# zubair-irshad/NeRF-MAE

Measured on AMD Instinct MI355X. Metric: voxel-grids/sec (fwd+bwd+optimizer) swin_s 160^3 bf16, higher is better.
Workload: dtype bf16; 1 GPU; swin_s MAE pretraining step, global batch 8 = 8 grid(s)/GPU of 4x160^3 RGB-sigma, mask_ratio 0.75, stochastic depth 0.1, AdamW+clip, DP=1 (BASELINE configs[2], the headline, read literally); global_batch=8, grids_per_gpu=8, resolution=160, parallelism=dp1, launch=hipgraph

## Files before the change

include/nerfmae_hip.h:

```cpp
#ifndef NERFMAE_HIP_H
#define NERFMAE_HIP_H
#include <stdint.h>
#ifdef __cplusplus
extern "C" {
#endif
#define NMH_API __attribute__((visibility("default")))

NMH_API int nmh_version(void);
NMH_API const char* nmh_error_string(int code);

NMH_API int nmh_gemm_nt(int dt, const void* A, int64_t lda, const void* W, int64_t ldw, int M, int N, int K, void* C, int64_t ldc, const float* bias, int act, void* C2, const void* resid, const float* rowscale, int rows_per_scale, int accumulate, void* stream);
NMH_API int nmh_gemm_nt_window_scatter(int dt, const void* A, int64_t lda, const void* W, int64_t ldw, int M, int N, int K, void* out, const void* resid, const float* bias, const float* rowscale, int tokens_per_sample, const int* wm, void* stream);
NMH_API int nmh_gemm_tn(int dt, const void* A, int64_t lda, const void* B, int64_t ldb, float* dW, int64_t M, int N, int K, const float* rowscale, int rows_per_scale, int omode, int64_t ldo, int p0, int p1, float* dbias, float* ws, int64_t ws_floats, void* stream);
typedef struct nmh_tn_problem { const void* A; int64_t lda; const void* B; int64_t ldb; float* dW; int64_t ldo; float* dbias; const float* rowscale; int64_t M; int N; int K; int rows_per_sample;
  int64_t stride_k; int up_k; int up_v; int bias_atomic; int n_inner; int64_t stride_n2; } nmh_tn_problem;
NMH_API int nmh_gemm_tn_grouped(int dt, const nmh_tn_problem* probs, int nprob, float* ws, int64_t ws_floats, void* stream);
NMH_API int nmh_gemm_tn_grouped_fg(int dt, const nmh_tn_problem* probs, int nprob, float* ws, int64_t ws_floats, void* stream);
NMH_API int nmh_conv3d_k3(int dt, const void* X, const void* Wp, void* Y, int B, int D, int H, int W, int Cin, int Cout, int accumulate, float* ws, int64_t ws_floats, void* stream);
NMH_API int nmh_conv3d_k3_bias(int dt, const void* X, const void* Wp, const float* bias, void* Y, int B, int D, int H, int W, int Cin, int Cout, void* stream);
NMH_API int nmh_nearest_upsample_add(int dt, const void* coarse, void* fine, int B, int Dc, int Hc, int Wc, int Df, int Hf, int Wf, int C, void* stream);
NMH_API int nmh_nearest_upsample_add_bwd(int dt, const void* dfine, void* dcoarse, int B, int Dc, int Hc, int Wc, int Df, int Hf, int Wf, int C, void* stream);
NMH_API int nmh_copy_cols(int dt, const void* src, int64_t lds, void* dst, int64_t ldd, int64_t M, int C, void* stream);
NMH_API int nmh_ndhwc_to_ncdhw(int dt, const void* src, float* dst, int B, int64_t V, int C, void* stream);
NMH_API int nmh_ncdhw_to_ndhwc(int dt, const float* src, void* dst, int B, int64_t V, int C, void* stream);
NMH_API int nmh_conv3d_k3_c48(const void* X, const void* Wk, void* Y, int B, int D, int H, int W, int accumulate, double* stats_acc, void* stream);
NMH_API int nmh_conv3d_k3_c48_bwd_reduce(const void* dY, const void* Wkd, void* dX, int B, int D, int H, int W, const void* Y1, const float* stats1, float slope, double* sums, void* stream);
NMH_API int nmh_conv3d_k3_c48mb(const void* X, const void* Wk, void* Y, int B, int D, int H, int W, int Cin, int Cout, int accumulate, void* stream);
NMH_API int nmh_conv3d_k3_c64(const void* X, const void* Wk, void* Y, int B, int D, int H, int W, int Cin, int Cout, int accumulate, double* stats_acc, const float* bias, void* stream);
NMH_API int64_t nmh_conv3d_k3_c64_pack_numel(int Cin, int Cout);
NMH_API int nmh_conv3d_k3_c64_wgrad(const void* dY, const void* X, float* dW, float* ws, int B, int D, int H, int W, int Cin, int Cout, void* stream);
NMH_API int64_t nmh_conv3d_k3_c64_wgrad_ws_floats(void);
NMH_API int nmh_instnorm_finalize(const double* acc, float* stats, int B, int64_t V, int C, float eps, void* stream);
NMH_API int nmh_conv3d_k3_c48_wgrad(const void* dY, const void* X, float* dW, float* ws, int B, int D, int H, int W, void* stream);
NMH_API int nmh_conv3d_k3_wgrad_halo(const void* dY, const void* X, float* dW, float* ws, int B, int D, int H, int W, int Cin, int Cout, void* stream);
NMH_API int64_t nmh_conv3d_k3_c48_wgrad_ws_floats(void);
NMH_API int nmh_conv3d_k3_wgrad(int dt, const void* dY, const void* X, float* dW, int B, int D, int H, int W, int Cin, int Cout, void* stream);

NMH_API int nmh_layernorm_fwd(int dt, int src_mode, const void* x, void* out, const float* gamma, const float* beta, float eps, float* mean, float* rstd, int64_t rows, int C, const int* wm, const float* pos, const unsigned char* mask, const float* mask_token, int64_t tokens_per_sample, void* stream);
NMH_API int nmh_layernorm_bwd(int dt, int src_mode, const void* dy, const void* x, const float* gamma, const float* mean, const float* rstd, const void* dres, void* dx, float* dgamma, float* dbeta, int64_t rows, int C, const int* wm, const unsigned char* mask, float* dmask_token, int64_t tokens_per_sample, void* dyw, const float* dyw_scale, void* stream);
typedef struct nmh_ln_reduce_item { const float* partials; float* dgamma; float* dbeta; int64_t partial_rows; int C; int reserved; } nmh_ln_reduce_item;
NMH_API int64_t nmh_layernorm_bwd_partial_rows(int64_t rows, int C);
NMH_API int nmh_layernorm_bwd_deferred(int dt, int src_mode, const void* dy, const void* x, const float* gamma, const float* mean, const float* rstd, const void* dres, void* dx, float* partials, int64_t rows, int C, const int* wm, void* dyw, const float* dyw_scale, int64_t tokens_per_sample, void* stream);
NMH_API int nmh_layernorm_param_grad_reduce(const nmh_ln_reduce_item* items, int n, void* stream);
NMH_API int64_t nmh_cconv_pack_numel(void);
NMH_API int64_t nmh_cconv_pack_ws_floats(void);
NMH_API int nmh_cconv_pack(const float* Wt, const float* W1, const float* bt, void* Wcp, float* delta, float* ws, void* stream);
NMH_API int nmh_cconv_fwd(const void* x, const void* Wcp, const float* delta, void* y1, int B, int v, double* stats_acc, void* stream);
NMH_API int nmh_cconv_pack_centered(const float* Wt, const float* W1, const float* bt, void* Wcp, float* delta, float* ws, float* mean_table, void* stream);
NMH_API int nmh_cconv_output_mean(const void* x, const float* mean_table, const float* delta, double* class_sums, float* mean, int B, int v, void* stream);
NMH_API int nmh_conv48_pack_scaled(const float* W, const float* stats, void* Wk_per_sample, int B, void* stream);
// ... 165 lines not shown
```

nerf-mae_amd/csrc/capi.hip:

```cpp
#include "../../include/nerfmae_hip.h"
#include "kernels.hpp"
#include <cstdio>

static inline WinMap to_wm(const int* w) {
  WinMap m{};
  if (w) { m.B = w[0]; m.H = w[1]; m.W = w[2]; m.D = w[3]; m.PH = w[4]; m.PW = w[5]; m.PD = w[6]; m.s0 = w[7]; m.s1 = w[8]; m.s2 = w[9]; }
  return m;
}
#define ST ((hipStream_t)stream)
#define NMH_DT_BF16_C 1
#define REQ(...) do { const void* req_[] = {__VA_ARGS__}; for (const void* q_ : req_) if (!q_) return -4; } while (0)
#define CLR() (void)hipGetLastError()

extern "C" {
int nmh_version(void) { return 100; }
const char* nmh_error_string(int code) {
  if (code == 0) return "ok";
  if (code == -1) return "nmh: unsupported operation";
  if (code == -2) return "nmh: shape constraint violated (channel counts must be multiples of 8; head_dim must be 32)";
  if (code == -3) return "nmh: row too wide for the layernorm kernels";
  if (code < 0) return "nmh: invalid argument";
  return hipGetErrorString((hipError_t)code);
}
int nmh_gemm_nt(int dt, const void* A, int64_t lda, const void* W, int64_t ldw, int M, int N, int K, void* C, int64_t ldc, const float* bias, int act, void* C2,
// ... 6 lines not shown
}
int nmh_gemm_nt_window_scatter(int dt, const void* A, int64_t lda, const void* W, int64_t ldw, int M, int N, int K, void* out, const void* resid, const float* bias,
                               const float* rowscale, int tokens_per_sample, const int* wm, void* stream) {
  CLR();
  REQ(A, W, out, resid, wm);
  if (M <= 0) return 0;
  EpiParams ep{out, N, bias, 0, nullptr, resid, rowscale, tokens_per_sample > 0 ? tokens_per_sample : 1, 0};
  ep.win_on = 1; ep.wm = to_wm(wm);
  return k_gemm_nt(dt, A, lda, W, ldw, M, N, K, ep, ST);
}
int nmh_gemm_tn(int dt, const void* A, int64_t lda, const void* B, int64_t ldb, float* dW, int64_t M, int N, int K, const float* rowscale, int rows_per_scale,
                int omode, int64_t ldo, int p0, int p1, float* dbias, float* ws, int64_t ws_floats, void* stream) {
  CLR();
  REQ(A, B, dW);
  if (M <= 0) return 0;
  TnGeom gm{};
  gm.omode = omode; gm.ldo = ldo; gm.dbias = dbias; gm.ws = ws; gm.ws_floats = ws ? (long)ws_floats : 0;
  if (omode == 2) { gm.Cin = p0; gm.V = (unsigned)p1; gm.dC = make_fdiv(p0); }
  return k_gemm_tn(dt, A, lda, B, ldb, dW, M, N, K, rowscale, rows_per_scale > 0 ? rows_per_scale : 1, gm, ST);
}
int nmh_gemm_tn_grouped(int dt, const nmh_tn_problem* probs, int nprob, float* ws, int64_t ws_floats, void* stream) {
  CLR();
  if (nprob <= 0) return 0;
  if (dt != NMH_DT_BF16_C || probs == nullptr) return -4;
  static_assert(sizeof(nmh_tn_problem) == sizeof(TnProblemHost), "descriptor layouts must agree");
  return k_gemm_tn_grouped(reinterpret_cast<const TnProblemHost*>(probs), nprob, ws, ws ? (long)ws_floats : 0, ST);
}
int nmh_gemm_tn_grouped_fg(int dt, const nmh_tn_problem* probs, int nprob, float* ws, int64_t ws_floats, void* stream) {
  CLR();
  if (nprob <= 0) return 0;
  if (dt != NMH_DT_BF16_C || probs == nullptr) return -4;
  return k_gemm_tn_grouped(reinterpret_cast<const TnProblemHost*>(probs), nprob, ws, ws ? (long)ws_floats : 0, ST, true);
}
int nmh_upconv_fwd(int dt, const void* x, const void* Wt, const float* bias, void* cat, int64_t ldc, int B, int v, int k, int Cin, int Cout, void* stream) {
  CLR();
  REQ(x, Wt, cat);
  return k_upconv_fwd(dt, x, Wt, bias, cat, (long)ldc, B, v, k, Cin, Cout, ST);
}
int nmh_upconv_dgrad(int dt, const void* dcat, int64_t ldc, const void* Wd, void* dx, int B, int v, int k, int Cin, int Cout, void* stream) {
  CLR();
  REQ(dcat, Wd, dx);
  return k_upconv_dgrad(dt, dcat, (long)ldc, Wd, dx, B, v, k, Cin, Cout, ST);
}
int nmh_upconv_wgrad(int dt, const void* dcat, int64_t ldc, const void* x, float* dW, float* dbias, int B, int v, int k, int Cin, int Cout, void* stream) {
  CLR();
  REQ(dcat, x, dW);
  return k_upconv_wgrad(dt, dcat, (long)ldc, x, dW, dbias, B, v, k, Cin, Cout, ST);
}
int nmh_conv3d_k3(int dt, const void* X, const void* Wp, void* Y, int B, int D, int H, int W, int Cin, int Cout, int accumulate, float* ws, int64_t ws_floats, void* stream) {
  CLR();
  REQ(X, Wp, Y);
  EpiParams ep{Y, Cout, nullptr, 0, nullptr, nullptr, nullptr, 1, accumulate};
  return k_conv3_nt(dt, X, Wp, B, D, H, W, Cin, Cout, ep, ST, ws, ws ? (long)ws_floats : 0);
}
int nmh_conv3d_k3_bias(int dt, const void* X, const void* Wp, const float* bias, void* Y, int B, int D, int H, int W, int Cin, int Cout, void* stream) {
  CLR();
  REQ(X, Wp, bias, Y);
  EpiParams ep{Y, Cout, bias, 0, nullptr, nullptr, nullptr, 1, 0};
  return k_conv3_nt(dt, X, Wp, B, D, H, W, Cin, Cout, ep, ST);
}
int nmh_conv3d_k3_c64(const void* X, const void* Wk, void* Y, int B, int D, int H, int W, int Cin, int Cout, int accumulate, double* stats_acc, const float* bias, void* stream) {
  CLR();
  if (!X || !Wk || !Y) return -4;
  return k_conv64(X, Wk, Y, B, D, H, W, Cin, Cout, accumulate, stats_acc, bias, ST);
}
int nmh_conv3d_k3_c64_wgrad(const void* dY, const void* X, float* dW, float* ws, int B, int D, int H, int W, int Cin, int Cout, void* stream) {
  CLR();
// ... 946 lines not shown
```

nerf-mae_amd/csrc/kernels.hpp:

```cpp
#pragma once
#include <hip/hip_runtime.h>

struct FDiv { unsigned M; int sh; unsigned d; };
FDiv make_fdiv(unsigned d);

struct WinMap { int B, H, W, D, PH, PW, PD, s0, s1, s2; };

struct EpiParams {
  void* C; long ldc;
  const float* bias;
  int act; void* C2;
  const void* resid;
  const float* rowscale; int rows_per_scale;
  int accumulate;
  int up_k, up_v, up_cout;
  FDiv up_dv, up_dk, up_dc;
  int win_on; WinMap wm;
  int ksplit; int nbatch; float* kpart;
};

struct TnGeom {
  int omode;
  long ldo;
  int Cin, D, H, W; unsigned V;
// ... 30 lines not shown
  const int x = (int)(tu - q * (unsigned)w.D);
  unsigned q2 = q / (unsigned)w.W;
  const int y = (int)(q - q2 * (unsigned)w.W);
  const unsigned b = q2 / (unsigned)w.H;
  const int z = (int)(q2 - b * (unsigned)w.H);
  int pz = z - w.s0, py = y - w.s1, px = x - w.s2;
  if (pz < 0) pz += w.PH;
  if (py < 0) py += w.PW;
  if (px < 0) px += w.PD;
  const unsigned win = ((b * ((unsigned)w.PH >> 2) + ((unsigned)pz >> 2)) * ((unsigned)w.PW >> 2) + ((unsigned)py >> 2)) * ((unsigned)w.PD >> 2) + ((unsigned)px >> 2);
  return (long)win * 64 + ((pz & 3) << 4) + ((py & 3) << 2) + (px & 3);
}

#endif
int k_gemm_nt(int dt, const void* A, long lda, const void* Bw, long ldb, int M, int N, int K, const EpiParams& ep, hipStream_t st);
int k_upconv_fwd(int dt, const void* x, const void* Wt, const float* bias, void* cat, long ldc, int B, int v, int k, int Cin, int Cout, hipStream_t st);
int k_upconv_dgrad(int dt, const void* dcat, long ldc, const void* Wd, void* dx, int B, int v, int k, int Cin, int Cout, hipStream_t st);
int k_upconv_wgrad(int dt, const void* dcat, long ldc, const void* x, float* dW, float* dbias, int B, int v, int k, int Cin, int Cout, hipStream_t st);
int k_conv3_nt(int dt, const void* X, const void* Wp, int B, int D, int H, int W, int Cin, int Cout, const EpiParams& ep, hipStream_t st, float* ws = nullptr, long ws_floats = 0);
int k_gemm_tn(int dt, const void* A, long lda, const void* Bm, long ldb, float* Out, long M, int N, int K, const float* rowscale, int rows_per_scale, const TnGeom& gm, hipStream_t st);
struct TnProblemHost {
  const void* A; long lda;
  const void* B; long ldb;
  float* dW; long ldo;
  float* dbias;
  const float* rowscale;
  long M; int N, K; int rows_per_sample;
  long stride_k;
  int up_k, up_v;
  int bias_atomic;
  int n_inner; long stride_n2;
};
int k_gemm_tn_grouped(const TnProblemHost* probs, int nprob, float* ws, long ws_floats, hipStream_t st, bool foreground = false);
int k_conv48(const void* X, const void* Wk, void* Y, int B, int D, int H, int W, int accumulate, double* stats_acc, hipStream_t st,
             const void* Y1 = nullptr, const float* stats1 = nullptr, float slope = 0.f, long wk_sample_stride = 0, int centered = 0);
int k_conv48_pack_scaled(const float* W, const float* stats, void* out, int B, hipStream_t st);
int k_conv48_mb(const void* X, const void* Wk, void* Y, int B, int D, int H, int W, int Cin, int Cout, int accumulate, hipStream_t st);
int k_conv64(const void* X, const void* Wk, void* Y, int B, int D, int H, int W, int Cin, int Cout, int accumulate, double* stats_acc, const float* bias, hipStream_t st);
long k_conv64_pack_numel(int Cin, int Cout);
int k_conv64_wgrad(const void* dY, const void* X, float* dW, float* ws, int B, int D, int H, int W, int Cin, int Cout, hipStream_t st);
long k_conv64_wgrad_ws_floats();
int k_in_finalize(int dt, const double* acc, float* stats, int B, long V, int C, float eps, hipStream_t st);
int k_conv48_wgrad(const void* dY, const void* X, float* dW, float* ws, int B, int D, int H, int W, hipStream_t st, const float* scale_stats = nullptr);
long k_conv48_wgrad_ws_floats();
int k_conv3_wgrad_halo(const void* dY, const void* X, float* dW, float* ws, int B, int D, int H, int W, int Cin, int Cout, hipStream_t st);
int k_conv3_tn(int dt, const void* dY, const void* X, float* dW, int B, int D, int H, int W, int Cin, int Cout, hipStream_t st);
int k_nearest_up_add(int dt, const void* coarse, void* fine, int B, int Dc, int Hc, int Wc, int Df, int Hf, int Wf, int C, int bwd, hipStream_t st);
int k_vc_transpose(int dt, const void* src, void* dst, int B, long V, int C, int dir, hipStream_t st);
int k_copy_cols(int dt, const void* src, long lds, void* dst, long ldd, long M, int C, hipStream_t st);

struct LnArgs {
  int dt; int src_mode;
  const void* x; void* out;
  const float* gamma; const float* beta; float eps;
  float* mean; float* rstd;
  long rows; int C;
  WinMap wm;
  const float* pos; const unsigned char* mask; const float* mask_token; long tokens_per_sample;
  void* out_tok;
  const int* rowmap; long cap_rows;
};
int k_ln_fwd(const LnArgs& a, hipStream_t st);
int k_mask_rowmap(const unsigned char* mask, int n, int cap, int* rowmap, hipStream_t st);
struct LnBwdArgs {
  int dt; int src_mode;
  const void* dy;
// ... 248 lines not shown
```

nerf-mae_amd/csrc/tn_grouped.hip:

```cpp
#include "common.hpp"
#include "kernels.hpp"
#include <algorithm>
#include <vector>

namespace tng {
constexpr int MAXP = 40;
constexpr int BN = 96, BK = 96, CH = 64, RS = 192, TILE = CH * RS, STAGE = 2 * TILE, ST = 2, PCS = 6;
constexpr int LDS_BYTES = ST * STAGE;

struct Prob {
  const bf16_t* A; const bf16_t* B; float* Out; float* dbias; const float* rowscale;
  int lda, ldb;
  int N, K;
  int rps, nsamp;
  int sub;
  int zs;
  int rbegin;
  int son, sok;
  int upflags;
  int partoff;
  int ncol2;
  __device__ __host__ int tk(int bt) const { return (K + bt - 1) / bt; }
  __device__ __host__ int ntile(int bt) const { return ((N + bt - 1) / bt) * tk(bt); }
  __device__ __host__ int mps() const { return ((rps + sub - 1) / sub + 63) / 64 * 64; }
// ... 2 lines not shown
  __device__ bool bias_atomic() const { return (upflags >> 8) & 1; }
  __device__ long out_off(int n, int k) const {
    if (ncol2) { const int ni = ncol2 & 0xffff, q = n / ni; return (long)(n - q * ni) * son + (long)q * (ncol2 >> 16) + (long)k * sok; }
    return (long)n * son + (long)k * sok;
  }
  __device__ int bias_col(int n) const { return ncol2 ? n % (ncol2 & 0xffff) : n; }
};
static_assert(sizeof(Prob) == 96, "kernel-argument budget");
struct Args { Prob p[MAXP]; int wbegin[MAXP]; float* ws; int nprob; int xcd; };
static_assert(sizeof(Args) <= 4096, "HIP kernel-argument segment");
}

__device__ uint4 g_zero16_tng[1];

__device__ __forceinline__ Frag<bf16_t> tng_frag(const char* tile, int m0, int col0, int lane) {
  const int g = lane >> 4, p = lane & 15;
  const int row = m0 + 4 * g + (p >> 2);
  const int ch = ((col0 >> 2) + (p & 3)) ^ (((row >> 2) & 1) << 2);
  const char* a = tile + row * tng::RS + ch * 8;
  bf16x4 lo = ds_read_tr16(a);
  bf16x4 hi = ds_read_tr16(a + 16 * tng::RS);
  Frag<bf16_t> f;
  f.v = __builtin_shufflevector(lo, hi, 0, 1, 2, 3, 4, 5, 6, 7);
  return f;
}

__device__ __forceinline__ unsigned tng_frag_ofs(int m0, int col0, int lane) {
  const int g = lane >> 4, p = lane & 15;
  const int row = m0 + 4 * g + (p >> 2);
  const int ch = ((col0 >> 2) + (p & 3)) ^ (((row >> 2) & 1) << 2);
  return (unsigned)(row * tng::RS + ch * 8);
}

template <bool RSC, bool BIG, bool REG>
__global__ __launch_bounds__(BIG ? 512 : 256) void gemm_tn_grouped_kernel(tng::Args ga) {
  using namespace tng;
  constexpr int NW = BIG ? 8 : 4, NSUB = BIG ? 4 : 2, BT = BIG ? 192 : 96, NB = BIG ? 6 : 3, STG = NSUB * TILE;
  extern __shared__ __attribute__((aligned(16))) char smem[];
  const int tid = threadIdx.x, lane = tid & 63, wave = __builtin_amdgcn_readfirstlane(tid >> 6), wn = wave >> 1, wk = wave & 1, g = lane >> 4, li = lane & 15;
  const int sa = BIG ? (wn >> 1) : 0, acol0 = (BIG ? (wn & 1) : wn) * 48, sb = BIG ? wk : 0, bcol0 = BIG ? 0 : wk * 48;
  int bid = (int)blockIdx.x;
  if (ga.xcd) {
    const int G = (int)gridDim.x, x = bid & 7, q = G >> 3, rem = G & 7;
    bid = x * q + (x < rem ? x : rem) + (bid >> 3);
  }
  int pi = 0;
#pragma unroll
  for (int i = 1; i < MAXP; ++i)
    if (bid >= ga.wbegin[i]) pi = i;
  const Prob& P = ga.p[pi];
  const int lw = bid - ga.wbegin[pi];
  const int ptk = P.tk(BT), pnt = P.ntile(BT), pmps = P.mps();
  float* const ppart = ga.ws + P.partoff;
  const int z = lw / pnt, t = lw - z * pnt;
  const int nt = t / ptk, kt = t - nt * ptk;
  const int n0 = nt * BT, k0 = kt * BT;
  const int N = P.N, K = P.K;
  const bf16_t* __restrict__ A = P.A;
  const bf16_t* __restrict__ Bm = P.B;
  const long lda = P.lda, ldb = P.ldb;
  const int up_k = P.up_k(), up_v = P.up_v();

  int s0, s1, sublo = 0, subhi = P.rps;
  if (P.zs == 1) { s0 = 0; s1 = P.nsamp; }
  else {
    const int b = z / P.sub, j = z - b * P.sub;
    s0 = b; s1 = b + 1;
    sublo = j * pmps;
    subhi = sublo + pmps < P.rps ? sublo + pmps : P.rps;
    if (sublo > subhi) sublo = subhi;
  }
  const int seglen = subhi - sublo;
  const int cps = (seglen + CH - 1) / CH;
  const int nc = cps * (s1 - s0);

  int prow[PCS], pcol[PCS], psub[PCS];
#pragma unroll
  for (int i = 0; i < PCS; ++i) {
    const int q = wave + NW * i, sub = q / 12, off = 1024 * (q - sub * 12) + 16 * lane;
    const int row = off / RS, u = (off - row * RS) >> 4;
    psub[i] = sub;
    prow[i] = row;
    pcol[i] = (u ^ (((row >> 2) & 1) << 1)) * 8 + (sub % (NSUB / 2)) * 96;
  }
  unsigned long long zpage = (unsigned long long)(const void*)g_zero16_tng;
  asm volatile("" : "+v"(zpage));
  int iseg = s0, ilc = 0, islot = 0;
  uint4 stg[REG ? PCS : 1];
  auto issue = [&]() {
    const long segbase = (long)iseg * P.rps + sublo;
    const int r0 = ilc * CH;
    char* slot = smem + islot * STG;
#pragma unroll
    for (int i = 0; i < PCS; ++i) {
      const int r = r0 + prow[i];
      const bool isA = BIG ? (psub[i] < NSUB / 2) : (i < 3);
      unsigned long long src = zpage;
      if (isA) {
        const int n = n0 + pcol[i];
        if (r < seglen && n < N) {
          long arow = segbase + r;
          if (up_k) {
            const unsigned vv = (unsigned)up_v, kk = (unsigned)up_k, m = (unsigned)arow;
            const unsigned q = m / vv, x = m - q * vv, q2 = q / vv, y = q - q2 * vv, bb = q2 / vv, zq = q2 - bb * vv;
            const long Vf = (long)vv * kk;
            arow = (((long)bb * Vf + zq * kk) * Vf + y * kk) * Vf + x * kk;
          }
          if (up_k && P.ncol2) {
            const int ni = P.ncol2 & 0xffff, q = n / ni;
            src = (unsigned long long)(A + (arow + q) * lda + (n - q * ni));
          } else src = (unsigned long long)(A + arow * lda + n);
        }
      } else {
        const int k = k0 + pcol[i];
        if (r < seglen && k < K) src = (unsigned long long)(Bm + (segbase + r) * ldb + k);
      }
      const int q = wave + NW * i;
      if constexpr (REG) stg[i] = src != zpage ? *reinterpret_cast<const uint4*>(src) : make_uint4(0, 0, 0, 0);
      else __builtin_amdgcn_global_load_lds((const __attribute__((address_space(1))) void*)src, (__attribute__((address_space(3))) void*)(slot + q * 1024), 16, 0, 0);
    }
    if (++ilc == cps) { ilc = 0; ++iseg; }
    if (!REG && ++islot == ST) islot = 0;
  };
  auto sstore = [&](int slotidx) {
#pragma unroll
    for (int i = 0; i < PCS; ++i) *reinterpret_cast<uint4*>(smem + slotidx * STG + (wave + NW * i) * 1024 + lane * 16) = stg[REG ? i : 0];
  };

  f32x4 acc[3][NB], tot[RSC ? 3 : 1][RSC ? NB : 1];
#pragma unroll
  for (int a = 0; a < 3; ++a)
#pragma unroll
    for (int b = 0; b < NB; ++b) {
      acc[a][b] = f32x4{0.f, 0.f, 0.f, 0.f};
      if (RSC) tot[RSC ? a : 0][RSC ? b : 0] = f32x4{0.f, 0.f, 0.f, 0.f};
    }
  const bool want_bias = P.dbias != nullptr && kt == 0 && wk == 0;
  f32x4 bacc[3], btot[RSC ? 3 : 1];
  Frag<bf16_t> ones;
#pragma unroll
  for (int a = 0; a < 3; ++a) { bacc[a] = f32x4{0.f, 0.f, 0.f, 0.f}; if (RSC) btot[RSC ? a : 0] = f32x4{0.f, 0.f, 0.f, 0.f}; }
#pragma unroll
  for (int j = 0; j < 8; ++j) ones.v[j] = (short)0x3F80;
  const bool scaled = RSC && P.rowscale != nullptr;

  unsigned aofs[3], bofs[NB];
#pragma unroll
  for (int a = 0; a < 3; ++a) aofs[a] = (unsigned)(sa * TILE) + tng_frag_ofs(0, acol0 + a * 16, lane);
#pragma unroll
  for (int b = 0; b < NB; ++b) bofs[b] = (unsigned)((NSUB / 2 + sb) * TILE) + tng_frag_ofs(0, bcol0 + b * 16, lane);
  const unsigned smem_u = lds_addr_u(smem);
  auto compute = [&](const char* stage) {
    if constexpr (REG) {
      const char* sA = stage + sa * TILE;
      const char* sB = stage + (NSUB / 2 + sb) * TILE;
#pragma unroll
      for (int s = 0; s < CH / 32; ++s) {
        Frag<bf16_t> bf[NB];
#pragma unroll
        for (int b = 0; b < NB; ++b) bf[b] = tng_frag(sB, s * 32, bcol0 + b * 16, lane);
#pragma unroll
        for (int a = 0; a < 3; ++a) {
          Frag<bf16_t> af = tng_frag(sA, s * 32, acol0 + a * 16, lane);
#pragma unroll
          for (int b = 0; b < NB; ++b) mma(acc[a][b], af, bf[b]);
          if (want_bias) mma(bacc[a], af, ones);
        }
      }
    } else {
      const unsigned st_u = smem_u + (unsigned)(stage - smem);
      TrFrag fb[2][NB], fa[2][3];
#pragma unroll
      for (int s = 0; s < CH / 32; ++s) {
#pragma unroll
        for (int b = 0; b < NB; ++b) tr_read_raw<16 * RS>(fb[s][b], st_u + bofs[b] + s * 32 * RS);
#pragma unroll
        for (int a = 0; a < 3; ++a) tr_read_raw<16 * RS>(fa[s][a], st_u + aofs[a] + s * 32 * RS);
      }
      tr_wait();
#pragma unroll
      for (int s = 0; s < CH / 32; ++s) {
#pragma unroll
        for (int b = 0; b < NB; ++b) tr_pin(fb[s][b]);
#pragma unroll
        for (int a = 0; a < 3; ++a) tr_pin(fa[s][a]);
      }
#pragma unroll
      for (int s = 0; s < CH / 32; ++s) {
#pragma unroll
        for (int a = 0; a < 3; ++a) {
          const Frag<bf16_t> af = tr_frag(fa[s][a]);
#pragma unroll
          for (int b = 0; b < NB; ++b) mma(acc[a][b], af, tr_frag(fb[s][b]));
          if (want_bias) mma(bacc[a], af, ones);
        }
      }
    }
  };
  int cseg = s0, clc = 0, cslot = 0;
  auto sample_end = [&]() {
    if (++clc == cps) {
      if (scaled) {
        const float sc = P.rowscale[cseg];
#pragma unroll
        for (int a = 0; a < 3; ++a) {
#pragma unroll
          for (int b = 0; b < NB; ++b) {
#pragma unroll
            for (int r = 0; r < 4; ++r) { tot[RSC ? a : 0][RSC ? b : 0][r] += sc * acc[a][b][r]; acc[a][b][r] = 0.f; }
          }
#pragma unroll
          for (int r = 0; r < 4; ++r) { btot[RSC ? a : 0][r] += sc * bacc[a][r]; bacc[a][r] = 0.f; }
        }
      }
      clc = 0; ++cseg;
    }
  };
  if constexpr (REG) {
    if (nc > 0) { issue(); sstore(0); }
    if (nc > 1) issue();
    __syncthreads();
    for (int c = 0; c < nc; ++c) {
      compute(smem + (c & 1) * STG);
      if (c + 1 < nc) {
        sstore((c + 1) & 1);
        if (c + 2 < nc) issue();
      }
      __syncthreads();
      sample_end();
    }
  } else {
#pragma unroll
    for (int s = 0; s < ST - 1; ++s)
      if (s < nc) issue();
    for (int c = 0; c < nc; ++c) {
      if (nc - 1 - c >= ST - 2) asm volatile("s_waitcnt vmcnt(%0)" ::"n"((ST - 2) * PCS) : "memory");
      else asm volatile("s_waitcnt vmcnt(0)" ::: "memory");
      __builtin_amdgcn_s_barrier();
      if (c + ST - 1 < nc) issue();
      compute(smem + cslot * STG);
      if (++cslot == ST) cslot = 0;
      sample_end();
    }
  }
#pragma unroll
  for (int a = 0; a < 3; ++a)
#pragma unroll
    for (int b = 0; b < NB; ++b)
#pragma unroll
      for (int r = 0; r < 4; ++r) {
        const int n = n0 + sa * 96 + acol0 + a * 16 + 4 * g + r, k = k0 + sb * 96 + bcol0 + b * 16 + li;
        if (n < N && k < K) {
          const float v = scaled ? tot[RSC ? a : 0][RSC ? b : 0][r] : acc[a][b][r];
          if (P.zs > 1) ppart[((long)z * N + n) * K + k] = v;
          else P.Out[P.out_off(n, k)] += v;
        }
      }
  if (want_bias && li == 0) {
#pragma unroll
    for (int a = 0; a < 3; ++a)
#pragma unroll
      for (int r = 0; r < 4; ++r) {
        const int n = n0 + sa * 96 + acol0 + a * 16 + 4 * g + r;
        if (n < N) {
          const float v = scaled ? btot[RSC ? a : 0][r] : bacc[a][r];
          if (P.zs > 1) ppart[(long)P.zs * N * K + (long)z * N + n] = v;
          else if (P.bias_atomic()) atomicAdd(P.dbias + P.bias_col(n), v);
          else P.dbias[P.bias_col(n)] += v;
        }
      }
  }
}

constexpr int TNG_RED_ITEMS = 64;
__global__ __launch_bounds__(256) void gemm_tn_grouped_reduce_kernel(tng::Args ga) {
  using namespace tng;
  int pi = -1;
#pragma unroll 1
  for (int i = 0; i < ga.nprob; ++i)
    if (ga.p[i].zs > 1 && (int)blockIdx.x >= ga.p[i].rbegin) pi = i;
  if (pi < 0) return;
  const Prob& P = ga.p[pi];
  const float* const ppart = ga.ws + P.partoff;
  const long NK = (long)P.N * P.K, NK4 = NK >> 2;
  const int lane = threadIdx.x & 63, wave = threadIdx.x >> 6, item = wave * 16 + (lane & 15), share = lane >> 4;
  const long i4 = (long)((int)blockIdx.x - P.rbegin) * TNG_RED_ITEMS + item;
  float4 s = make_float4(0.f, 0.f, 0.f, 0.f);
  const bool is_w = i4 < NK4, is_b = !is_w && P.dbias && i4 < NK4 + P.N;
  if (is_w) {
    const float* src = ppart + i4 * 4;
    int z = share;
    for (; z + 12 < P.zs; z += 16) {
      const float4 v0 = *reinterpret_cast<const float4*>(src + (long)z * NK), v1 = *reinterpret_cast<const float4*>(src + (long)(z + 4) * NK);
      const float4 v2 = *reinterpret_cast<const float4*>(src + (long)(z + 8) * NK), v3 = *reinterpret_cast<const float4*>(src + (long)(z + 12) * NK);
      s.x += (v0.x + v1.x) + (v2.x + v3.x); s.y += (v0.y + v1.y) + (v2.y + v3.y); s.z += (v0.z + v1.z) + (v2.z + v3.z); s.w += (v0.w + v1.w) + (v2.w + v3.w);
    }
    for (; z < P.zs; z += 4) {
      const float4 v = *reinterpret_cast<const float4*>(src + (long)z * NK);
// ... 297 lines not shown
        p.rbegin = rb;
        rb += (int)(((long)p.N * p.K / 4 + (p.dbias ? p.N : 0) + TNG_RED_ITEMS - 1) / TNG_RED_ITEMS);
      }
      if (!fits) {
        for (int i = 0; i < np; ++i) rest.push_back(idx[base + i]);
        continue;
      }
      if (int e = (cu & 1) ? tns::launch_cfg<true>(c, ga, w, st) : tns::launch_cfg<false>(c, ga, w, st)) return e;
      hipLaunchKernelGGL(gemm_tn_grouped_reduce_kernel, dim3(rb), dim3(256), 0, st, ga);
      NMH_CHECK_LAUNCH();
      ntaken += np;
    }
  }
  return ntaken;
}

static int k_gemm_tn_grouped_tiles(const TnProblemHost* probs, int nprob, float* ws, long ws_floats, hipStream_t st, bool foreground);
int k_gemm_tn_grouped(const TnProblemHost* probs, int nprob, float* ws, long ws_floats, hipStream_t st, bool foreground) {
  std::vector<int> rest;
  const int taken = tn_stream_launches(probs, nprob, rest, ws, ws_floats, st, foreground);
  if (taken < 0) return taken;
  if (taken == 0) return k_gemm_tn_grouped_tiles(probs, nprob, ws, ws_floats, st, foreground);
  if (rest.empty()) return 0;
  std::vector<TnProblemHost> r(rest.size());
  for (size_t i = 0; i < rest.size(); ++i) r[i] = probs[rest[i]];
  return k_gemm_tn_grouped_tiles(r.data(), (int)r.size(), ws, ws_floats, st, foreground);
}
static int k_gemm_tn_grouped_tiles(const TnProblemHost* probs, int nprob, float* ws, long ws_floats, hipStream_t st, bool foreground) {
  using namespace tng;
  static NmhPerDeviceOnce attr_set;
  if (attr_set.need()) {
    hipError_t e = hipSuccess;
    auto setattr = [&](const void* f, int bytes) { if (e == hipSuccess) e = hipFuncSetAttribute(f, hipFuncAttributeMaxDynamicSharedMemorySize, bytes); };
    setattr((const void*)gemm_tn_grouped_kernel<false, false, false>, LDS_BYTES);
    setattr((const void*)gemm_tn_grouped_kernel<true, false, false>, LDS_BYTES);
    setattr((const void*)gemm_tn_grouped_kernel<false, true, false>, 2 * LDS_BYTES);
    setattr((const void*)gemm_tn_grouped_kernel<true, true, false>, 2 * LDS_BYTES);
    setattr((const void*)gemm_tn_grouped_kernel<false, true, true>, 2 * 4 * TILE);
    setattr((const void*)gemm_tn_grouped_kernel<true, true, true>, 2 * 4 * TILE);
    if (e != hipSuccess) return (int)e;
    attr_set.set();
  }
  static const int target_bg = getenv("NMH_TNG_TARGET") ? atoi(getenv("NMH_TNG_TARGET")) : 256;
  static const int target_fg = getenv("NMH_TNG_TARGET_FG") ? atoi(getenv("NMH_TNG_TARGET_FG")) : 640;
  const int target_wgs = foreground ? target_fg : target_bg;
  static const int flat_tiles = getenv("NMH_TNG_FLAT") ? atoi(getenv("NMH_TNG_FLAT")) : 384;
  std::vector<int> order(nprob);
  for (int i = 0; i < nprob; ++i) order[i] = i;
  std::stable_sort(order.begin(), order.end(), [&](int a, int b) { return probs[a].M > probs[b].M; });
  const int nlaunch = (nprob + MAXP - 1) / MAXP, per = (nprob + nlaunch - 1) / nlaunch;
  for (int base = 0; base < nprob; base += per) {
    const int np = std::min(per, nprob - base);
    Args ga{};
    ga.nprob = np;
    ga.ws = ws;
    static const int xcd_map = getenv("NMH_TNG_XCD") ? atoi(getenv("NMH_TNG_XCD")) : 1;
    ga.xcd = xcd_map;
    long tiles = 0, tiles_big = 0;
    bool any_rs = false, all192 = true;
    for (int i = 0; i < np; ++i) {
      const TnProblemHost& h = probs[order[base + i]];
      if (h.K % 8 || h.lda % 8 || h.ldb % 8 || h.rows_per_sample <= 0 || h.M % h.rows_per_sample || !h.A || !h.B || !h.dW) return -4;
      if (h.up_k > 0 && (h.up_v <= 0 || h.up_k > 255 || h.up_v > 65535 || h.rows_per_sample != (long)h.up_v * h.up_v * h.up_v)) return -4;
      if (h.lda >= (1L << 31) || h.ldb >= (1L << 31) || h.ldo >= (1L << 31) || h.stride_k >= (1L << 31)) return -4;
      Prob& p = ga.p[i];
      p.A = (const bf16_t*)h.A; p.B = (const bf16_t*)h.B; p.Out = h.dW; p.dbias = h.dbias; p.rowscale = h.rowscale;
      p.lda = (int)h.lda; p.ldb = (int)h.ldb; p.N = h.N; p.K = h.K;
      p.son = (int)h.ldo; p.sok = h.stride_k > 0 ? (int)h.stride_k : 1;
      if (h.n_inner < 0 || h.n_inner > 65535 || (h.n_inner > 0 && (h.stride_n2 < 0 || h.stride_n2 > 32767 || h.N % h.n_inner))) return -4;
      p.ncol2 = h.n_inner > 0 ? (h.n_inner | ((int)h.stride_n2 << 16)) : 0;
      p.upflags = (h.up_k & 0xff) | ((h.bias_atomic || h.n_inner > 0 ? 1 : 0) << 8)    | (h.up_k > 0 ? (h.up_v << 16) : 0);
      p.rps = h.rows_per_sample; p.nsamp = (int)(h.M / h.rows_per_sample);
      tiles += p.ntile(96);
      tiles_big += p.ntile(192);
      all192 &= h.N % 192 == 0 && h.K % 192 == 0;
      any_rs |= h.rowscale != nullptr;
    }
    const int big_min = getenv("NMH_TNG_BIG") ? atoi(getenv("NMH_TNG_BIG")) : 0;
    const bool big = big_min > 0 && all192 && tiles_big >= big_min;
    const int bt = big ? 192 : 96;
    if (big) tiles = tiles_big;
    int S = tiles >= flat_tiles ? 1 : (int)((target_wgs + tiles - 1) / tiles);
    long wsoff = 0;
    int w = 0, rb = 0;
    bool any_split = false;
    for (int i = 0; i < MAXP; ++i) ga.wbegin[i] = 0x7fffffff;
    for (int i = 0; i < np; ++i) {
      Prob& p = ga.p[i];
      p.zs = 1; p.sub = 1; p.partoff = 0;
      if (S > 1) {
        int sub = (S + p.nsamp - 1) / p.nsamp;
        const int maxsub = std::max(1, p.rps / 1024);
        sub = std::max(1, std::min(sub, maxsub));
        int zs = p.nsamp * sub;
        const long need = (long)zs * p.N * (p.K + 1);
        if (zs > 1 && ws && wsoff + need <= ws_floats && wsoff + need < (1L << 31)) {
          p.zs = zs; p.sub = sub;
          p.partoff = (int)wsoff;
          wsoff += (need + 3) / 4 * 4;
          any_split = true;
        }
      }
      ga.wbegin[i] = w;
      w += p.ntile(bt) * p.zs;
      p.rbegin = rb;
      if (p.zs > 1) rb += (int)(((long)p.N * p.K / 4 + (p.dbias ? p.N : 0) + TNG_RED_ITEMS - 1) / TNG_RED_ITEMS);
    }
    const int reg_stage = getenv("NMH_TNG_REG") ? atoi(getenv("NMH_TNG_REG")) : 0;
    if (reg_stage) {
      if (big) {
        if (any_rs) hipLaunchKernelGGL((gemm_tn_grouped_kernel<true, true, true>), dim3(w), dim3(512), 2 * 4 * TILE, st, ga);
        else hipLaunchKernelGGL((gemm_tn_grouped_kernel<false, true, true>), dim3(w), dim3(512), 2 * 4 * TILE, st, ga);
      } else {
        if (any_rs) hipLaunchKernelGGL((gemm_tn_grouped_kernel<true, false, true>), dim3(w), dim3(256), 2 * 2 * TILE, st, ga);
        else hipLaunchKernelGGL((gemm_tn_grouped_kernel<false, false, true>), dim3(w), dim3(256), 2 * 2 * TILE, st, ga);
      }
    } else if (big) {
      if (any_rs) hipLaunchKernelGGL((gemm_tn_grouped_kernel<true, true, false>), dim3(w), dim3(512), 2 * LDS_BYTES, st, ga);
      else hipLaunchKernelGGL((gemm_tn_grouped_kernel<false, true, false>), dim3(w), dim3(512), 2 * LDS_BYTES, st, ga);
    } else {
      if (any_rs) hipLaunchKernelGGL((gemm_tn_grouped_kernel<true, false, false>), dim3(w), dim3(256), LDS_BYTES, st, ga);
      else hipLaunchKernelGGL((gemm_tn_grouped_kernel<false, false, false>), dim3(w), dim3(256), LDS_BYTES, st, ga);
    }
    NMH_CHECK_LAUNCH();
    if (any_split) {
      hipLaunchKernelGGL(gemm_tn_grouped_reduce_kernel, dim3(rb), dim3(256), 0, st, ga);
      NMH_CHECK_LAUNCH();
    }
  }
  return 0;
}
```

nerf-mae_amd/ops.py:

```python
from __future__ import annotations

import ctypes
from typing import Optional, Sequence

import torch

from ._lib import lib

F32, BF16 = 0, 1
WS = 4
PROFILE = None
PROFILE_BYTES = {}


def _prof(key, nbytes=None):
    if PROFILE is None:
        return None
    if nbytes is not None:
        PROFILE_BYTES[key] = nbytes
    a, b = torch.cuda.Event(enable_timing=True), torch.cuda.Event(enable_timing=True)
    PROFILE.setdefault(key, []).append((a, b))
    a.record(torch.cuda.current_stream())
    return b

# ... 118 lines not shown
                ("K", ctypes.c_int), ("rows_per_sample", ctypes.c_int), ("stride_k", ctypes.c_int64), ("up_k", ctypes.c_int), ("up_v", ctypes.c_int),
                ("bias_atomic", ctypes.c_int), ("n_inner", ctypes.c_int), ("stride_n2", ctypes.c_int64)]


GROUPED_WGRAD = __import__("os").environ.get("NMH_TNG", "1") != "0"
DEFER_DECODER_WGRAD = __import__("os").environ.get("NMH_DEFER_DEC", "1") == "1"
WQ_FLUSH_AFTER_FIRST = __import__("os").environ.get("NMH_WQ_FLUSH_AFTER_FIRST", "1") == "1"


class _LnReduceItem(ctypes.Structure):
    _fields_ = [("partials", ctypes.c_void_p), ("dgamma", ctypes.c_void_p), ("dbeta", ctypes.c_void_p), ("partial_rows", ctypes.c_int64), ("C", ctypes.c_int),
                ("reserved", ctypes.c_int)]


def ln_param_grad_reduce(items):
    group, seen = [], set()

    def launch(g):
        if not g:
            return
        arr = (_LnReduceItem * len(g))()
        for i, (part, nb, C, dg, db) in enumerate(g):
            _chk(part, dg, db)
            arr[i] = _LnReduceItem(part.data_ptr(), dg.data_ptr(), db.data_ptr(), nb, C, 0)
        lib().call("nmh_layernorm_param_grad_reduce", arr, len(g), _st())

    for it in items:
        if it[3].data_ptr() in seen:
            launch(group)
            group, seen = [], set()
        group.append(it)
        seen.add(it[3].data_ptr())
    launch(group)


class WgradQueue:

    def __init__(self):
        self.pending, self.inflight, self._cb, self.sync_after_flush = [], [], False, False
        self.ln_items = []
        self.pad_items = {}
        self.deferred = []
        self._due = False

    def reset(self):
        if self.pending or self.deferred or self.inflight or self._cb:
            join_side()
            self.pending, self.deferred, self.inflight, self._cb, self._due = [], [], [], False, False
            self.ln_items, self.pad_items = [], {}

    def defer(self, fn):
        self.deferred.append(fn)
        if not self._cb:
            self._cb = True
            torch.autograd.Variable._execution_engine.queue_callback(self._final)

    def add_ln_partials(self, part, nb, C, dgamma, dbeta):
        if not self.ln_items:
            items = self.ln_items = []
            self.defer(lambda: ln_param_grad_reduce(items))
        self.ln_items.append((part, nb, C, dgamma, dbeta))

    def add_pad_colsum(self, x, out, geom):
        key = (tuple(geom.carr), x.shape[1], x.dtype)
        groups = self.pad_items
        if key not in groups:
# ... 1973 lines not shown
```

Measured before the change: 194.6 grids/s.

## Fold rowscale into running accumulator and skip zero-scale samples in grouped wgrad GEMM

Removes the separate per-sample total accumulators in the grouped TN weight-gradient kernel. At each sample boundary the accumulator is rescaled by the ratio of consecutive row scales, and the final scale is applied once at writeout. Samples whose rowscale is zero (stochastic-depth-dropped) are skipped entirely when loading and computing. Launch bounds now request 2 or 3 workgroups per CU, and a residency query API is added. This cuts register pressure and redundant work, at the cost of extra floating-point rounding from repeated ratio rescaling and possible spills forced by the tighter launch bounds.

Result: no change. 195.2 grids/s, median of 6 (+0.3%).

```diff
diff --git a/include/nerfmae_hip.h b/include/nerfmae_hip.h
--- a/include/nerfmae_hip.h
+++ b/include/nerfmae_hip.h
@@ -16,6 +16,7 @@
   int64_t stride_k; int up_k; int up_v; int bias_atomic; int n_inner; int64_t stride_n2; } nmh_tn_problem;
 NMH_API int nmh_gemm_tn_grouped(int dt, const nmh_tn_problem* probs, int nprob, float* ws, int64_t ws_floats, void* stream);
 NMH_API int nmh_gemm_tn_grouped_fg(int dt, const nmh_tn_problem* probs, int nprob, float* ws, int64_t ws_floats, void* stream);
+NMH_API int nmh_gemm_tn_grouped_residency(int* wgs_per_cu);
 NMH_API int nmh_conv3d_k3(int dt, const void* X, const void* Wp, void* Y, int B, int D, int H, int W, int Cin, int Cout, int accumulate, float* ws, int64_t ws_floats, void* stream);
 NMH_API int nmh_conv3d_k3_bias(int dt, const void* X, const void* Wp, const float* bias, void* Y, int B, int D, int H, int W, int Cin, int Cout, void* stream);
 NMH_API int nmh_nearest_upsample_add(int dt, const void* coarse, void* fine, int B, int Dc, int Hc, int Wc, int Df, int Hf, int Wf, int C, void* stream);
diff --git a/nerf-mae_amd/csrc/capi.hip b/nerf-mae_amd/csrc/capi.hip
--- a/nerf-mae_amd/csrc/capi.hip
+++ b/nerf-mae_amd/csrc/capi.hip
@@ -62,7 +62,12 @@
   if (dt != NMH_DT_BF16_C || probs == nullptr) return -4;
   return k_gemm_tn_grouped(reinterpret_cast<const TnProblemHost*>(probs), nprob, ws, ws ? (long)ws_floats : 0, ST, true);
 }
-int nmh_upconv_fwd(int dt, const void* x, const void* Wt, const float* bias, void* cat, int64_t ldc, int B, int v, int k, int Cin, int Cout, void* stream) {
+int nmh_gemm_tn_grouped_residency(int* wgs_per_cu) {
+  CLR();
+  REQ(wgs_per_cu);
+  return k_gemm_tn_grouped_residency(wgs_per_cu);
+}
+int nmh_upconv_fwd(int dt, const void* x,const void* Wt, const float* bias, void* cat, int64_t ldc, int B, int v, int k, int Cin, int Cout, void* stream) {
   CLR();
   REQ(x, Wt, cat);
   return k_upconv_fwd(dt, x, Wt, bias, cat, (long)ldc, B, v, k, Cin, Cout, ST);
diff --git a/nerf-mae_amd/csrc/kernels.hpp b/nerf-mae_amd/csrc/kernels.hpp
--- a/nerf-mae_amd/csrc/kernels.hpp
+++ b/nerf-mae_amd/csrc/kernels.hpp
@@ -86,6 +86,7 @@
   int n_inner; long stride_n2;
 };
 int k_gemm_tn_grouped(const TnProblemHost* probs, int nprob, float* ws, long ws_floats, hipStream_t st, bool foreground = false);
+int k_gemm_tn_grouped_residency(int* wgs_per_cu);
 int k_conv48(const void* X, const void* Wk, void* Y, int B, int D, int H, int W, int accumulate, double* stats_acc, hipStream_t st,
              const void* Y1 = nullptr, const float* stats1 = nullptr, float slope = 0.f, long wk_sample_stride = 0, int centered = 0);
 int k_conv48_pack_scaled(const float* W, const float* stats, void* out, int B, hipStream_t st);
diff --git a/nerf-mae_amd/csrc/tn_grouped.hip b/nerf-mae_amd/csrc/tn_grouped.hip
--- a/nerf-mae_amd/csrc/tn_grouped.hip
+++ b/nerf-mae_amd/csrc/tn_grouped.hip
@@ -58,8 +58,9 @@
   return (unsigned)(row * tng::RS + ch * 8);
 }
 
-template <bool RSC, bool BIG, bool REG>
-__global__ __launch_bounds__(BIG ? 512 : 256) void gemm_tn_grouped_kernel(tng::Args ga) {
+template <bool BIG, bool REG>
+__global__ __launch_bounds__(BIG ? 512 : 256, BIG ? 2 : 3)
+void gemm_tn_grouped_kernel(tng::Args ga) {
   using namespace tng;
   constexpr int NW = BIG ? 8 : 4, NSUB = BIG ? 4 : 2, BT = BIG ? 192 : 96, NB = BIG ? 6 : 3, STG = NSUB * TILE;
   extern __shared__ __attribute__((aligned(16))) char smem[];
@@ -98,7 +99,15 @@
   }
   const int seglen = subhi - sublo;
   const int cps = (seglen + CH - 1) / CH;
-  const int nc = cps * (s1 - s0);
+  const float* __restrict__ rsc = P.rowscale;
+  auto next_live = [&](int s) {
+    if (rsc != nullptr)
+      while (s < s1 && rsc[s] == 0.f) ++s;
+    return s;
+  };
+  int nlive = 0;
+  for (int s = next_live(s0); s < s1; s = next_live(s + 1)) ++nlive;
+  const int nc = cps * nlive;
 
   int prow[PCS], pcol[PCS], psub[PCS];
 #pragma unroll
@@ -111,7 +120,7 @@
   }
   unsigned long long zpage = (unsigned long long)(const void*)g_zero16_tng;
   asm volatile("" : "+v"(zpage));
-  int iseg = s0, ilc = 0, islot = 0;
+  int iseg = next_live(s0), ilc = 0, islot = 0;
   uint4 stg[REG ? PCS : 1];
   auto issue = [&]() {
     const long segbase = (long)iseg * P.rps + sublo;
@@ -145,7 +154,7 @@
       if constexpr (REG) stg[i] = src != zpage ? *reinterpret_cast<const uint4*>(src) : make_uint4(0, 0, 0, 0);
       else __builtin_amdgcn_global_load_lds((const __attribute__((address_space(1))) void*)src, (__attribute__((address_space(3))) void*)(slot + q * 1024), 16, 0, 0);
     }
-    if (++ilc == cps) { ilc = 0; ++iseg; }
+    if (++ilc == cps) { ilc = 0; iseg = next_live(iseg + 1); }
     if (!REG && ++islot == ST) islot = 0;
   };
   auto sstore = [&](int slotidx) {
@@ -153,22 +162,20 @@
     for (int i = 0; i < PCS; ++i) *reinterpret_cast<uint4*>(smem + slotidx * STG + (wave + NW * i) * 1024 + lane * 16) = stg[REG ? i : 0];
   };
 
-  f32x4 acc[3][NB], tot[RSC ? 3 : 1][RSC ? NB : 1];
+  f32x4 acc[3][NB];
 #pragma unroll
   for (int a = 0; a < 3; ++a)
 #pragma unroll
-    for (int b = 0; b < NB; ++b) {
-      acc[a][b] = f32x4{0.f, 0.f, 0.f, 0.f};
-      if (RSC) tot[RSC ? a : 0][RSC ? b : 0] = f32x4{0.f, 0.f, 0.f, 0.f};
-    }
+    for (int b = 0; b < NB; ++b) acc[a][b] = f32x4{0.f, 0.f, 0.f, 0.f};
   const bool want_bias = P.dbias != nullptr && kt == 0 && wk == 0;
-  f32x4 bacc[3], btot[RSC ? 3 : 1];
+  f32x4 bacc[3];
   Frag<bf16_t> ones;
 #pragma unroll
-  for (int a = 0; a < 3; ++a) { bacc[a] = f32x4{0.f, 0.f, 0.f, 0.f}; if (RSC) btot[RSC ? a : 0] = f32x4{0.f, 0.f, 0.f, 0.f}; }
+  for (int a = 0; a < 3; ++a) bacc[a] = f32x4{0.f, 0.f, 0.f, 0.f};
 #pragma unroll
   for (int j = 0; j < 8; ++j) ones.v[j] = (short)0x3F80;
-  const bool scaled = RSC && P.rowscale != nullptr;
+  const bool scaled = rsc != nullptr;
+  float endscale = scaled ? 0.f : 1.f;
 
   unsigned aofs[3], bofs[NB];
 #pragma unroll
@@ -223,23 +230,28 @@
       }
     }
   };
-  int cseg = s0, clc = 0, cslot = 0;
+  int cseg = next_live(s0), clc = 0, cslot = 0;
   auto sample_end = [&]() {
     if (++clc == cps) {
+      const int nseg = next_live(cseg + 1);
       if (scaled) {
-        const float sc = P.rowscale[cseg];
-#pragma unroll
-        for (int a = 0; a < 3; ++a) {
-#pragma unroll
-          for (int b = 0; b < NB; ++b) {
-#pragma unroll
-            for (int r = 0; r < 4; ++r) { tot[RSC ? a : 0][RSC ? b : 0][r] += sc * acc[a][b][r]; acc[a][b][r] = 0.f; }
+        endscale = rsc[cseg];
+        if (nseg < s1) {
+          const float ratio = endscale / rsc[nseg];
+          if (ratio != 1.0f) {
+#pragma unroll
+            for (int a = 0; a < 3; ++a) {
+#pragma unroll
+              for (int b = 0; b < NB; ++b)
+#pragma unroll
+                for (int r = 0; r < 4; ++r) acc[a][b][r] *= ratio;
+#pragma unroll
+              for (int r = 0; r < 4; ++r) bacc[a][r] *= ratio;
+            }
           }
-#pragma unroll
-          for (int r = 0; r < 4; ++r) { btot[RSC ? a : 0][r] += sc * bacc[a][r]; bacc[a][r] = 0.f; }
         }
       }
-      clc = 0; ++cseg;
+      clc = 0; cseg = nseg;
     }
   };
   if constexpr (REG) {
@@ -277,7 +289,7 @@
       for (int r = 0; r < 4; ++r) {
         const int n = n0 + sa * 96 + acol0 + a * 16 + 4 * g + r, k = k0 + sb * 96 + bcol0 + b * 16 + li;
         if (n < N && k < K) {
-          const float v = scaled ? tot[RSC ? a : 0][RSC ? b : 0][r] : acc[a][b][r];
+          const float v = scaled ? endscale * acc[a][b][r] : acc[a][b][r];
           if (P.zs > 1) ppart[((long)z * N + n) * K + k] = v;
           else P.Out[P.out_off(n, k)] += v;
         }
@@ -289,7 +301,7 @@
       for (int r = 0; r < 4; ++r) {
         const int n = n0 + sa * 96 + acol0 + a * 16 + 4 * g + r;
         if (n < N) {
-          const float v = scaled ? btot[RSC ? a : 0][r] : bacc[a][r];
+          const float v = scaled ? endscale * bacc[a][r] : bacc[a][r];
           if (P.zs > 1) ppart[(long)P.zs * N * K + (long)z * N + n] = v;
           else if (P.bias_atomic()) atomicAdd(P.dbias + P.bias_col(n), v);
           else P.dbias[P.bias_col(n)] += v;
@@ -653,12 +665,9 @@
   if (attr_set.need()) {
     hipError_t e = hipSuccess;
     auto setattr = [&](const void* f, int bytes) { if (e == hipSuccess) e = hipFuncSetAttribute(f, hipFuncAttributeMaxDynamicSharedMemorySize, bytes); };
-    setattr((const void*)gemm_tn_grouped_kernel<false, false, false>, LDS_BYTES);
-    setattr((const void*)gemm_tn_grouped_kernel<true, false, false>, LDS_BYTES);
-    setattr((const void*)gemm_tn_grouped_kernel<false, true, false>, 2 * LDS_BYTES);
-    setattr((const void*)gemm_tn_grouped_kernel<true, true, false>, 2 * LDS_BYTES);
-    setattr((const void*)gemm_tn_grouped_kernel<false, true, true>, 2 * 4 * TILE);
-    setattr((const void*)gemm_tn_grouped_kernel<true, true, true>, 2 * 4 * TILE);
+    setattr((const void*)gemm_tn_grouped_kernel<false, false>, LDS_BYTES);
+    setattr((const void*)gemm_tn_grouped_kernel<true, false>, 2 * LDS_BYTES);
+    setattr((const void*)gemm_tn_grouped_kernel<true, true>, 2 * 4 * TILE);
     if (e != hipSuccess) return (int)e;
     attr_set.set();
   }
@@ -678,7 +687,7 @@
     static const int xcd_map = getenv("NMH_TNG_XCD") ? atoi(getenv("NMH_TNG_XCD")) : 1;
     ga.xcd = xcd_map;
     long tiles = 0, tiles_big = 0;
-    bool any_rs = false, all192 = true;
+    bool all192 = true;
     for (int i = 0; i < np; ++i) {
       const TnProblemHost& h = probs[order[base + i]];
       if (h.K % 8 || h.lda % 8 || h.ldb % 8 || h.rows_per_sample <= 0 || h.M % h.rows_per_sample || !h.A || !h.B || !h.dW) return -4;
@@ -695,7 +704,6 @@
       tiles += p.ntile(96);
       tiles_big += p.ntile(192);
       all192 &= h.N % 192 == 0 && h.K % 192 == 0;
-      any_rs |= h.rowscale != nullptr;
     }
     const int big_min = getenv("NMH_TNG_BIG") ? atoi(getenv("NMH_TNG_BIG")) : 0;
     const bool big = big_min > 0 && all192 && tiles_big >= big_min;
@@ -729,20 +737,10 @@
     }
     const int reg_stage = getenv("NMH_TNG_REG") ? atoi(getenv("NMH_TNG_REG")) : 0;
     if (reg_stage) {
-      if (big) {
-        if (any_rs) hipLaunchKernelGGL((gemm_tn_grouped_kernel<true, true, true>), dim3(w), dim3(512), 2 * 4 * TILE, st, ga);
-        else hipLaunchKernelGGL((gemm_tn_grouped_kernel<false, true, true>), dim3(w), dim3(512), 2 * 4 * TILE, st, ga);
-      } else {
-        if (any_rs) hipLaunchKernelGGL((gemm_tn_grouped_kernel<true, false, true>), dim3(w), dim3(256), 2 * 2 * TILE, st, ga);
-        else hipLaunchKernelGGL((gemm_tn_grouped_kernel<false, false, true>), dim3(w), dim3(256), 2 * 2 * TILE, st, ga);
-      }
-    } else if (big) {
-      if (any_rs) hipLaunchKernelGGL((gemm_tn_grouped_kernel<true, true, false>), dim3(w), dim3(512), 2 * LDS_BYTES, st, ga);
-      else hipLaunchKernelGGL((gemm_tn_grouped_kernel<false, true, false>), dim3(w), dim3(512), 2 * LDS_BYTES, st, ga);
-    } else {
-      if (any_rs) hipLaunchKernelGGL((gemm_tn_grouped_kernel<true, false, false>), dim3(w), dim3(256), LDS_BYTES, st, ga);
-      else hipLaunchKernelGGL((gemm_tn_grouped_kernel<false, false, false>), dim3(w), dim3(256), LDS_BYTES, st, ga);
-    }
+      if (big) hipLaunchKernelGGL((gemm_tn_grouped_kernel<true, true>), dim3(w), dim3(512), 2 * 4 * TILE, st, ga);
+      else hipLaunchKernelGGL((gemm_tn_grouped_kernel<false, true>), dim3(w), dim3(256), 2 * 2 * TILE, st, ga);
+    } else if (big) hipLaunchKernelGGL((gemm_tn_grouped_kernel<true, false>), dim3(w), dim3(512), 2 * LDS_BYTES, st, ga);
+    else hipLaunchKernelGGL((gemm_tn_grouped_kernel<false, false>), dim3(w), dim3(256), LDS_BYTES, st, ga);
     NMH_CHECK_LAUNCH();
     if (any_split) {
       hipLaunchKernelGGL(gemm_tn_grouped_reduce_kernel, dim3(rb), dim3(256), 0, st, ga);
@@ -751,3 +749,7 @@
   }
   return 0;
 }
+
+int k_gemm_tn_grouped_residency(int* wgs_per_cu) {
+  return (int)hipOccupancyMaxActiveBlocksPerMultiprocessor(wgs_per_cu, (const void*)gemm_tn_grouped_kernel<false, false>, 256, tng::LDS_BYTES);
+}
diff --git a/nerf-mae_amd/ops.py b/nerf-mae_amd/ops.py
--- a/nerf-mae_amd/ops.py
+++ b/nerf-mae_amd/ops.py
@@ -174,6 +174,12 @@
         group.append(it)
         seen.add(it[3].data_ptr())
     launch(group)
+
+
+def gemm_tn_grouped_residency() -> int:
+    n = (ctypes.c_int * 1)()
+    lib().call("nmh_gemm_tn_grouped_residency", n)
+    return int(n[0])
 
 
 class WgradQueue:
```
